# zifeo/distributed-sgd

Hardware: NVIDIA H100
Metric: sgd_samples_per_sec (higher is better)
Workload: dtype f64

## Files before the change

### distributed_sgd_b200/csrc/dsgd_api.cu

```cuda
#include "../../include/dsgd.h"

#include <cuda_runtime.h>
#include <dlfcn.h>
#include <nccl.h>

#include <algorithm>
#include <cstdarg>
#include <cstdio>
#include <cstring>
#include <string>
#include <vector>

#include "dsgd_kernels.cuh"
#include "dsgd_persistent.cuh"
#include "dsgd_stream.cuh"
#include "dsgd_async.cuh"
#include <cstdlib>

using namespace dsgd;

struct dsgd_ctx {
  int device = 0;
  int32_t dim = 0;
  double lambda = 0.0;
// ... 10 lines not shown
  int64_t n_rows = 0, nnz = 0, n_pairs = 0;
  bool rows_unique = false;
  uint32_t *rp16 = nullptr;
  uint2 *pairs = nullptr;
  int8_t *label = nullptr;
  float *yabs = nullptr;

  double *w = nullptr, *g = nullptr, *d = nullptr, *w_req = nullptr;
  float *w32 = nullptr, *w32_req = nullptr;
  unsigned long long *n_exact = nullptr;
  bool stream_ready = false;
  double *scal = nullptr;
  unsigned long long *cnt = nullptr;
  double *partial = nullptr;
  double *out2 = nullptr;
  double *gsum = nullptr;
  std::vector<int32_t> worker_counts;
  int32_t n_local = 1, k_total = 0;
  bool have_d = false;

  int32_t *samples = nullptr;
  int64_t samples_cap = 0, samples_n = 0;
  double *losses = nullptr;
  int64_t losses_cap = 0;
  double *preds = nullptr;
  int64_t preds_cap = 0;

  ncclComm_t comm = nullptr;

  double *p_wbuf[2] = {nullptr, nullptr};
  double *p_gbuf[3] = {nullptr, nullptr, nullptr};
  double2 *p_rec[3] = {nullptr, nullptr, nullptr};
  unsigned long long *p_acc = nullptr;
  unsigned *p_hinge = nullptr;
  int64_t p_hinge_cap = 0;
  unsigned *p_bar = nullptr;
  bool p_ready = false;
  long long *p_tl = nullptr;

  cudaStream_t astream = nullptr;
  cudaStream_t stream2 = nullptr;
  double *m_w = nullptr;
  double *outbox = nullptr;
  double *peer_w[kMaxReplicas] = {};
  bool peer_ipc[kMaxReplicas] = {};
  int *a_stop = nullptr;
  unsigned long long *a_cnt = nullptr;
  double *a_scratch = nullptr;
  int64_t a_scratch_lanes = 0;
  int32_t *a_rows = nullptr, *a_assigned = nullptr, *a_replay = nullptr;
  int64_t a_rows_cap = 0, a_assigned_cap = 0, a_replay_cap = 0;
  int32_t *u_idx = nullptr; double *u_val = nullptr; int64_t u_cap = 0;
  bool a_running = false;
  cudaEvent_t a_ev0 = nullptr, a_ev1 = nullptr;

  double *xblk = nullptr;
  double *peer_x[kMaxWorld] = {};
  bool peer_x_ipc[kMaxWorld] = {};
  int grid_limit = 0;
  int64_t x_step = 0;
  int64_t x_steps_run = 0;
  unsigned long long *x_llw = nullptr;
  unsigned long long *x_stats = nullptr;

  int32_t prof_every = 0;
  int64_t prof_seen = 0;
  std::vector<std::pair<cudaEvent_t, cudaEvent_t>> prof_events;
  size_t prof_used = 0;

  mutable std::string err;
  mutable std::string info;
};

static thread_local std::string g_create_err;

struct nccl_api {
  ncclResult_t (*GetUniqueId)(ncclUniqueId *) = nullptr;
  ncclResult_t (*CommInitRank)(ncclComm_t *, int, ncclUniqueId, int) = nullptr;
  ncclResult_t (*AllReduce)(const void *, void *, size_t, ncclDataType_t, ncclRedOp_t, ncclComm_t, cudaStream_t) = nullptr;
  ncclResult_t (*CommDestroy)(ncclComm_t) = nullptr;
  const char *(*GetErrorString)(ncclResult_t) = nullptr;
  bool ok = false;
  std::string why;
};
static nccl_api &nccl() {
  static nccl_api api = [] {
    nccl_api a;
    void *h = dlopen("libnccl.so.2", RTLD_NOW | RTLD_NOLOAD);
    if (!h)
      if (const char *p = getenv("DSGD_NCCL_PATH")) h = dlopen(p, RTLD_NOW | RTLD_GLOBAL);
    if (!h) h = dlopen("libnccl.so.2", RTLD_NOW | RTLD_GLOBAL);
    if (!h) { a.why = std::string("cannot load libnccl.so.2: ") + dlerror(); return a; }
// ... 111 lines not shown
  if ((e = cudaMalloc(&ctx->out2, sizeof(double) * 8)) != cudaSuccess) return bail("cudaMalloc out2", e);
  if ((e = cudaMalloc(&ctx->gsum, vd)) != cudaSuccess) return bail("cudaMalloc gsum", e);
  cudaMemsetAsync(ctx->gsum, 0, vd, ctx->stream);
  cudaMemsetAsync(ctx->w, 0, vd, ctx->stream);
  cudaMemsetAsync(ctx->g, 0, vd, ctx->stream);
  cudaMemsetAsync(ctx->d, 0, vd, ctx->stream);
  cudaMemsetAsync(ctx->w_req, 0, vd, ctx->stream);
  cudaMemsetAsync(ctx->w32, 0, sizeof(float) * (size_t)(dim + 2), ctx->stream);
  cudaMemsetAsync(ctx->scal, 0, sizeof(double) * kNumScal, ctx->stream);
  cudaMemsetAsync(ctx->cnt, 0, sizeof(unsigned long long) * kNumCnt, ctx->stream);
  if ((e = cudaStreamSynchronize(ctx->stream)) != cudaSuccess) return bail("init memset", e);
  *out = ctx;
  return DSGD_OK;
}

extern "C" int dsgd_destroy(dsgd_ctx *ctx) {
  if (!ctx) return DSGD_OK;
  cudaSetDevice(ctx->device);
  cudaDeviceSynchronize();
  if (ctx->comm) nccl().CommDestroy(ctx->comm);
  for (int r = 0; r < kMaxReplicas; ++r)
    if (ctx->peer_w[r] && ctx->peer_ipc[r]) cudaIpcCloseMemHandle(ctx->peer_w[r]);
  for (int r = 0; r < kMaxWorld; ++r)
    if (ctx->peer_x[r] && ctx->peer_x_ipc[r]) cudaIpcCloseMemHandle(ctx->peer_x[r]);
  if (ctx->xblk) cudaFree(ctx->xblk);
  if (ctx->x_llw) cudaFree(ctx->x_llw);
  void *aptrs[] = {ctx->m_w, ctx->outbox, ctx->a_stop, ctx->a_cnt, ctx->a_scratch, ctx->a_rows, ctx->a_assigned, ctx->a_replay, ctx->u_idx, ctx->u_val};
  for (void *q : aptrs) if (q) cudaFree(q);
  if (ctx->a_ev0) { cudaEventDestroy(ctx->a_ev0); cudaEventDestroy(ctx->a_ev1); }
  if (ctx->astream) cudaStreamDestroy(ctx->astream);
  if (ctx->stream2) cudaStreamDestroy(ctx->stream2);
  void *ptrs[] = {ctx->rp16, ctx->pairs, ctx->label, ctx->yabs, ctx->w, ctx->g, ctx->d, ctx->w_req, ctx->w32, ctx->w32_req, ctx->n_exact, ctx->scal,
                  ctx->cnt, ctx->partial, ctx->out2, ctx->gsum, ctx->p_wbuf[0], ctx->p_wbuf[1], ctx->p_gbuf[0],
                  ctx->p_gbuf[1], ctx->p_gbuf[2], ctx->p_rec[0], ctx->p_rec[1], ctx->p_rec[2], ctx->p_acc, ctx->p_hinge, ctx->p_bar, ctx->x_stats, ctx->samples,
                  ctx->losses, ctx->preds};
  for (void *p : ptrs) if (p) cudaFree(p);
  if (ctx->ev0) cudaEventDestroy(ctx->ev0);
  if (ctx->ev1) cudaEventDestroy(ctx->ev1);
  for (auto &pe : ctx->prof_events) { cudaEventDestroy(pe.first); cudaEventDestroy(pe.second); }
  if (ctx->own_stream) cudaStreamDestroy(ctx->own_stream);
  delete ctx;
  return DSGD_OK;
}

extern "C" const char *dsgd_last_error(const dsgd_ctx *ctx) { return ctx ? ctx->err.c_str() : g_create_err.c_str(); }

extern "C" const char *dsgd_info(const dsgd_ctx *ctx) {
  if (!ctx) return "{}";
  char buf[512];
  snprintf(buf, sizeof buf,
           "{\"device\": %d, \"name\": \"%s\", \"sm_count\": %d, \"arch\": \"sm_90a\", \"dim\": %d, \"rank\": %d, "
           "\"world\": %d, \"n_rows\": %lld, \"nnz\": %lld, \"state_dtype\": \"f64\", \"value_dtype\": \"f32\"}",
           ctx->device, ctx->dev_name.c_str(), ctx->sm_count, ctx->dim, ctx->rank, ctx->world, (long long)ctx->n_rows,
           (long long)ctx->nnz);
  ctx->info = buf;
  return ctx->info.c_str();
}

extern "C" int dsgd_set_stream(dsgd_ctx *ctx, void *cuda_stream) {
  if (!ctx) return DSGD_ERR_INVALID;
  CU(cudaSetDevice(ctx->device));
  CU(cudaStreamSynchronize(ctx->stream));
  ctx->stream = cuda_stream ? (cudaStream_t)cuda_stream : ctx->own_stream;
  return DSGD_OK;
}

extern "C" int dsgd_synchronize(dsgd_ctx *ctx) {
// ... 396 lines not shown
  CU(cudaSetDevice(ctx->device));
  CU(cudaStreamSynchronize(ctx->stream));
  CU(cudaMemcpy(&host, ctx->n_exact, sizeof host, cudaMemcpyDeviceToHost));
  *rows = (int64_t)host;
  return DSGD_OK;
}


extern "C" int dsgd_comm_unique_id(uint8_t id[DSGD_UNIQUE_ID_BYTES]) {
  static_assert(sizeof(ncclUniqueId) == DSGD_UNIQUE_ID_BYTES, "ncclUniqueId size");
  if (!id) return DSGD_ERR_INVALID;
  if (!nccl().ok) return fail(nullptr, DSGD_ERR_NCCL, "%s", nccl().why.c_str());
  ncclUniqueId u;
  ncclResult_t r = nccl().GetUniqueId(&u);
  if (r != ncclSuccess) return fail(nullptr, DSGD_ERR_NCCL, "ncclGetUniqueId: %s", nccl().GetErrorString(r));
  memcpy(id, &u, sizeof u);
  return DSGD_OK;
}

extern "C" int dsgd_comm_init(dsgd_ctx *ctx, const uint8_t id[DSGD_UNIQUE_ID_BYTES]) {
  if (!ctx) return DSGD_ERR_INVALID;
  NEED(id, DSGD_ERR_INVALID, "dsgd_comm_init: id is NULL");
  NEED(!ctx->comm, DSGD_ERR_STATE, "dsgd_comm_init: communicator already initialised");
  CU(cudaSetDevice(ctx->device));
  ncclUniqueId u;
  memcpy(&u, id, sizeof u);
  NEED(nccl().ok, DSGD_ERR_NCCL, "%s", nccl().why.c_str());
  NC(nccl().CommInitRank(&ctx->comm, ctx->world, u, ctx->rank));
  return DSGD_OK;
}

constexpr int kPCons = 8, kPUpd = 6, kPStages = 8, kPStagePairs = 2560, kPMaxChunks = 128;
using PSmem = PersistSmem<kPCons, kPUpd, kPStages, kPStagePairs, kPMaxChunks>;
#define DSGD_PERSIST_KERNEL(multi) k_sync_persistent<kPCons, kPUpd, kPStages, kPStagePairs, kPMaxChunks, multi>
static bool persist_timeline() { static const bool v = getenv("DSGD_PERSIST_TIMELINE") != nullptr; return v; }

static int persist_prepare(dsgd_ctx *ctx, int64_t n_steps) {
  if (!ctx->p_ready) {
    const size_t vd = sizeof(double) * (size_t)(ctx->dim + 2);
    for (int i = 0; i < 2; ++i) CU(cudaMalloc(&ctx->p_wbuf[i], vd));
    for (int i = 0; i < 3; ++i) {
      CU(cudaMalloc(&ctx->p_gbuf[i], vd));
      CU(cudaMemsetAsync(ctx->p_gbuf[i], 0, vd, ctx->stream));
      CU(cudaMalloc(&ctx->p_rec[i], 2 * vd));
      CU(cudaMemsetAsync(ctx->p_rec[i], 0, 2 * vd, ctx->stream));
    }
    CU(cudaMalloc(&ctx->p_acc, sizeof(unsigned long long) * 3 * kAccStride));
    CU(cudaMalloc(&ctx->p_bar, sizeof(unsigned) * 4));
    CU(cudaFuncSetAttribute((const void *)DSGD_PERSIST_KERNEL(false), cudaFuncAttributeMaxDynamicSharedMemorySize, (int)sizeof(PSmem)));
    CU(cudaFuncSetAttribute((const void *)DSGD_PERSIST_KERNEL(true), cudaFuncAttributeMaxDynamicSharedMemorySize, (int)sizeof(PSmem)));
    ctx->p_ready = true;
  }
  if (ctx->p_hinge_cap < n_steps) {
    if (ctx->p_hinge) CU(cudaFree(ctx->p_hinge));
    ctx->p_hinge = nullptr;
    const int64_t want = std::max<int64_t>(n_steps, 4096);
    CU(cudaMalloc(&ctx->p_hinge, sizeof(unsigned) * (size_t)want));
    ctx->p_hinge_cap = want;
  }
  return DSGD_OK;
}

static int persist_grid(const dsgd_ctx *ctx, int64_t batch) {
  const int g = ctx->grid_limit > 0 ? std::min(ctx->grid_limit, ctx->sm_count) : ctx->sm_count;
  if (cdiv(batch, kMaxRowsPerCta) > g) return 0;
  if (ctx->n_pairs >= (1ll << 31)) return 0;
  return g;
}
static bool persist_multi_fits(const dsgd_ctx *ctx, int G) {
  const int slice = (cdiv(ctx->dim + 1, G) + 31) & ~31;
  return slice <= (kPCons + kPUpd) * 32;
}

static cudaError_t persist_launch(dsgd_ctx *ctx, void *fn, int G, void **args) {
  if (ctx->grid_limit > 0) return cudaLaunchKernel(fn, dim3(G), dim3((kPCons + kPUpd + 1) * 32), args, sizeof(PSmem), ctx->stream);
  return cudaLaunchCooperativeKernel(fn, dim3(G), dim3((kPCons + kPUpd + 1) * 32), args, sizeof(PSmem), ctx->stream);
}

static int persist_params(dsgd_ctx *ctx, PersistParams &pp, const int32_t *samples_dev, int64_t n_per_step, int64_t n_steps,
                          double lr, double *losses_dev, int G) {
  (void)G;
  memset(&pp, 0, sizeof pp);
  pp.rp16 = ctx->rp16; pp.pairs = ctx->pairs; pp.label = ctx->label; pp.samples = samples_dev;
  pp.n_steps = n_steps; pp.batch = (int32_t)n_per_step; pp.dim = ctx->dim;
  pp.wbuf[0] = ctx->p_wbuf[0]; pp.wbuf[1] = ctx->p_wbuf[1];
  for (int i = 0; i < 3; ++i) { pp.gbuf[i] = ctx->p_gbuf[i]; pp.rec[i] = ctx->p_rec[i]; }
  pp.d = ctx->d; pp.acc = ctx->p_acc; pp.bar = ctx->p_bar; pp.hinge = ctx->p_hinge; pp.losses = losses_dev;
  pp.w_out = ctx->w; pp.w32_out = ctx->w32; pp.scal = ctx->scal;
  pp.abort_flag = reinterpret_cast<int *>(ctx->p_bar + 1);
  CU(cudaMemsetAsync(ctx->p_acc, 0, sizeof(unsigned long long) * 3 * kAccStride, ctx->stream));
  pp.lambda = ctx->lambda; pp.lr = lr; pp.world = 1;
  CU(cudaMemsetAsync(ctx->p_hinge, 0, sizeof(unsigned) * (size_t)n_steps, ctx->stream));
  CU(cudaMemsetAsync(ctx->p_bar, 0, sizeof(unsigned) * 4, ctx->stream));
  if (persist_timeline()) {
    if (!ctx->p_tl) CU(cudaMalloc(&ctx->p_tl, sizeof(long long) * kTlWords));
    CU(cudaMemsetAsync(ctx->p_tl, 0, sizeof(long long) * kTlWords, ctx->stream));
    pp.tl = ctx->p_tl;
  }
  return DSGD_OK;
}

static int persist_run(dsgd_ctx *ctx, const int32_t *samples_dev, int64_t n_per_step, int64_t n_steps, double lr,
                       double *losses_dev) {
  int rc = persist_prepare(ctx, n_steps);
  if (rc) return rc;
  const int G = persist_grid(ctx, n_per_step);
  NEED((uint64_t)G * (uint64_t)(n_steps + 2) < (1ull << 32), DSGD_ERR_INVALID, "dsgd_sync_steps: too many steps for one launch");
  PersistParams pp;
  if ((rc = persist_params(ctx, pp, samples_dev, n_per_step, n_steps, lr, losses_dev, G))) return rc;
  k_rec_init<<<cdiv(ctx->dim, 256), 256, 0, ctx->stream>>>(ctx->w, ctx->dim, ctx->p_rec[0], ctx->p_rec[1], ctx->p_rec[2]);
  LAUNCHED();
  pp.k_den = 1.0;
  pp.timeout_cycles = 4000000000ll;
  void *args[] = {&pp};
  auto *pe = prof_slot(ctx);
  if (pe) cudaEventRecord(pe->first, ctx->stream);
  CU(persist_launch(ctx, (void *)DSGD_PERSIST_KERNEL(false), G, args));
  if (pe) cudaEventRecord(pe->second, ctx->stream);
  LAUNCHED();
  return DSGD_OK;
}

static size_t xblk_stride(const dsgd_ctx *ctx) { return (size_t)(ctx->dim + kReplicaPad); }
static size_t xblk_words(const dsgd_ctx *ctx) { return ((size_t)ctx->dim + 1 + 31) / 32; }
static size_t xblk_bm_offset(const dsgd_ctx *ctx) { return 2 * (size_t)kMaxWorld * 2 * xblk_stride(ctx); }
static size_t xblk_doubles(const dsgd_ctx *ctx) { return xblk_bm_offset(ctx) + (size_t)kMaxWorld * 2 * xblk_words(ctx); }

static int xblk_ensure(dsgd_ctx *ctx) {
  if (ctx->xblk) return DSGD_OK;
  CU(cudaSetDevice(ctx->device));
  CU(cudaMalloc(&ctx->xblk, sizeof(double) * xblk_doubles(ctx)));
  CU(cudaMemset(ctx->xblk, 0, sizeof(double) * xblk_doubles(ctx)));
  CU(cudaMalloc(&ctx->x_stats, sizeof(unsigned long long) * 4));
  CU(cudaMemset(ctx->x_stats, 0, sizeof(unsigned long long) * 4));
  return DSGD_OK;
}

static int xllw_ensure(dsgd_ctx *ctx) {
  if (ctx->x_llw) return DSGD_OK;
  CU(cudaMalloc(&ctx->x_llw, 2 * 2 * sizeof(unsigned long long) * xblk_stride(ctx)));
  CU(cudaMemsetAsync(ctx->x_llw, 0, 2 * 2 * sizeof(unsigned long long) * xblk_stride(ctx), ctx->stream));
  return DSGD_OK;
}

static bool xchg_complete(const dsgd_ctx *ctx) {
  if (ctx->world <= 1 || ctx->world > kMaxWorld || !ctx->xblk) return false;
  for (int r = 0; r < ctx->world; ++r)
    if (r != ctx->rank && !ctx->peer_x[r]) return false;
  return true;
}

static int persist_run_multi(dsgd_ctx *ctx, const int32_t *samples_dev, int64_t n_per_step, int64_t n_steps, double lr,
                             double *losses_dev) {
  int rc = persist_prepare(ctx, n_steps);
  if (rc) return rc;
  const int G = persist_grid(ctx, n_per_step);
  NEED((uint64_t)G * (uint64_t)(n_steps + 2) < (1ull << 32), DSGD_ERR_INVALID, "dsgd_sync_steps: too many steps for one launch");
  PersistParams pp;
  if ((rc = persist_params(ctx, pp, samples_dev, n_per_step, n_steps, lr, losses_dev, G))) return rc;
  CU(cudaMemcpyAsync(ctx->p_wbuf[0], ctx->w, sizeof(double) * (size_t)ctx->dim, cudaMemcpyDeviceToDevice, ctx->stream));
  pp.k_den = (double)ctx->world;
  pp.timeout_cycles = 20000000000ll;
  pp.world = ctx->world; pp.rank = ctx->rank; pp.step_base = ctx->x_step;
  pp.xstride = (int)xblk_stride(ctx);
  pp.xwords = (int)xblk_words(ctx);
  for (int r = 0; r < ctx->world; ++r) {
    unsigned long long *blk = reinterpret_cast<unsigned long long *>((r == ctx->rank) ? ctx->xblk : ctx->peer_x[r]);
    pp.xval[r] = blk;
    pp.xbm[r] = blk + xblk_bm_offset(ctx);
  }
  if ((rc = xllw_ensure(ctx))) return rc;
  pp.llw[0] = ctx->x_llw;
  pp.llw[1] = ctx->x_llw + 2 * xblk_stride(ctx);
  pp.xstats = ctx->x_stats;
  void *args[] = {&pp};
  auto *pe = prof_slot(ctx);
  if (pe) cudaEventRecord(pe->first, ctx->stream);
  CU(persist_launch(ctx, (void *)DSGD_PERSIST_KERNEL(true), G, args));
  if (pe) cudaEventRecord(pe->second, ctx->stream);
  LAUNCHED();
  ctx->x_step += n_steps + 6;
  ctx->x_steps_run += n_steps;
  return DSGD_OK;
}

extern "C" int dsgd_reserve(dsgd_ctx *ctx, int64_t n_samples, int64_t n_steps) {
  if (!ctx) return DSGD_ERR_INVALID;
  NEED(n_samples >= 0 && n_steps >= 0, DSGD_ERR_INVALID, "dsgd_reserve: negative size");
  CU(cudaSetDevice(ctx->device));
  int rc = ensure_i32(ctx, &ctx->samples, &ctx->samples_cap, n_samples);
  if (rc) return rc;
  if ((rc = ensure_f64(ctx, &ctx->losses, &ctx->losses_cap, n_steps))) return rc;
  if ((rc = persist_prepare(ctx, n_steps))) return rc;
  if (persist_timeline() && !ctx->p_tl) CU(cudaMalloc(&ctx->p_tl, sizeof(long long) * kTlWords));
  if (ctx->world > 1 && !(ctx->flags & DSGD_FLAG_ASYNC)) {
    if ((rc = xblk_ensure(ctx))) return rc;
    if ((rc = xllw_ensure(ctx))) return rc;
  }
  CU(cudaStreamSynchronize(ctx->stream));
  return DSGD_OK;
}

extern "C" int dsgd_set_grid_limit(dsgd_ctx *ctx, int32_t n_ctas) {
  if (!ctx) return DSGD_ERR_INVALID;
  NEED(n_ctas >= 0, DSGD_ERR_INVALID, "dsgd_set_grid_limit: negative");
  ctx->grid_limit = n_ctas;
  return DSGD_OK;
}

extern "C" int dsgd_xchg_stats(dsgd_ctx *ctx, int64_t *value_words, int64_t *bitmap_words, int64_t *steps) {
  if (!ctx) return DSGD_ERR_INVALID;
  unsigned long long host[2] = {0, 0};
  if (ctx->x_stats) {
    CU(cudaSetDevice(ctx->device));
    CU(cudaStreamSynchronize(ctx->stream));
    CU(cudaMemcpy(host, ctx->x_stats, sizeof host, cudaMemcpyDeviceToHost));
  }
  if (value_words) *value_words = (int64_t)host[0];
  if (bitmap_words) *bitmap_words = (int64_t)host[1];
  if (steps) *steps = ctx->x_steps_run;
  return DSGD_OK;
}

extern "C" int dsgd_xchg_export(dsgd_ctx *ctx, uint8_t handle[DSGD_IPC_HANDLE_BYTES]) {
  if (!ctx || !handle) return DSGD_ERR_INVALID;
  NEED(!(ctx->flags & DSGD_FLAG_ASYNC), DSGD_ERR_STATE, "dsgd_xchg_export: ctx is in async mode");
// ... 10 lines not shown
  NEED(peer_rank >= 0 && peer_rank < ctx->world && peer_rank < kMaxWorld && peer_rank != ctx->rank, DSGD_ERR_INVALID,
       "dsgd_xchg_import: bad peer rank %d", peer_rank);
  int rc = xblk_ensure(ctx);
  if (rc) return rc;
  cudaIpcMemHandle_t h;
  memcpy(&h, handle, sizeof h);
  void *ptr = nullptr;
  CU(cudaIpcOpenMemHandle(&ptr, h, cudaIpcMemLazyEnablePeerAccess));
  if (ctx->peer_x[peer_rank] && ctx->peer_x_ipc[peer_rank]) cudaIpcCloseMemHandle(ctx->peer_x[peer_rank]);
  ctx->peer_x[peer_rank] = static_cast<double *>(ptr);
  ctx->peer_x_ipc[peer_rank] = true;
  return DSGD_OK;
}

extern "C" int dsgd_xchg_attach(dsgd_ctx *ctx, int peer_rank, dsgd_ctx *peer) {
  if (!ctx || !peer) return DSGD_ERR_INVALID;
  NEED(peer_rank >= 0 && peer_rank < ctx->world && peer_rank < kMaxWorld && peer_rank != ctx->rank, DSGD_ERR_INVALID,
       "dsgd_xchg_attach: bad peer rank %d", peer_rank);
  NEED(peer->dim == ctx->dim, DSGD_ERR_INVALID, "dsgd_xchg_attach: dimension mismatch");
  int rc = xblk_ensure(ctx);
  if (rc) return rc;
  if ((rc = xblk_ensure(peer))) { ctx->err = peer->err; return rc; }
  CU(cudaSetDevice(ctx->device));
  if (peer->device != ctx->device) {
    int can = 0;
    CU(cudaDeviceCanAccessPeer(&can, ctx->device, peer->device));
    NEED(can, DSGD_ERR_CUDA, "dsgd_xchg_attach: device %d cannot access device %d", ctx->device, peer->device);
    cudaError_t e = cudaDeviceEnablePeerAccess(peer->device, 0);
    if (e != cudaSuccess && e != cudaErrorPeerAccessAlreadyEnabled) CU(e);
    (void)cudaGetLastError();
  }
  ctx->peer_x[peer_rank] = peer->xblk;
  ctx->peer_x_ipc[peer_rank] = false;
  return DSGD_OK;
}

static int persist_check(dsgd_ctx *ctx) {
  if (!ctx->p_ready) return DSGD_OK;
  unsigned host[2] = {0, 0};
  CU(cudaMemcpy(host, ctx->p_bar, sizeof host, cudaMemcpyDeviceToHost));
  NEED(host[1] == 0, DSGD_ERR_TIMEOUT, "persistent sync kernel: a device-side wait (grid barrier, peer word) hit its watchdog");
  return DSGD_OK;
}

static_assert(kTlWords == DSGD_TIMELINE_WORDS, "timeline layout");
extern "C" int dsgd_debug_timeline(dsgd_ctx *ctx, long long *out) {
  if (!ctx || !out) return DSGD_ERR_INVALID;
  NEED(ctx->p_tl, DSGD_ERR_STATE, "no timeline recorded (set DSGD_PERSIST_TIMELINE=1)");
  CU(cudaStreamSynchronize(ctx->stream));
  CU(cudaMemcpy(out, ctx->p_tl, sizeof(long long) * kTlWords, cudaMemcpyDeviceToHost));
  return DSGD_OK;
}

extern "C" int dsgd_set_workers(dsgd_ctx *ctx, int32_t n_local, const int32_t *counts, int32_t k_total) {
  if (!ctx) return DSGD_ERR_INVALID;
  NEED(n_local >= 0 && k_total >= 0, DSGD_ERR_INVALID, "dsgd_set_workers: negative count");
  NEED(n_local <= 1 || counts, DSGD_ERR_INVALID, "dsgd_set_workers: counts is NULL");
  std::vector<int32_t> c;
  if (counts)
    for (int32_t v = 0; v < n_local; ++v) {
      NEED(counts[v] > 0, DSGD_ERR_EMPTY, "dsgd_set_workers: worker %d has an empty batch (Vec.sum of an empty list throws)", v);
      c.push_back(counts[v]);
    }
  ctx->worker_counts = c;
  ctx->n_local = n_local;
  ctx->k_total = k_total;
// ... 394 lines not shown
```

### distributed_sgd_b200/csrc/dsgd_persistent.cuh

```cuda
#pragma once
#include <cuda_runtime.h>
#include <stdint.h>

#include "dsgd_kernels.cuh"

namespace dsgd {

constexpr int kMaxWorld = 8;

struct PersistParams {
  const uint32_t *rp16;
  const uint2 *pairs;
  const int8_t *label;
  const int32_t *samples;
  int64_t n_steps;
  int32_t batch;
  int32_t dim;
  double *wbuf[2];
  double *gbuf[3];
  double2 *rec[3];
  const double *d;
  unsigned long long *acc;
  unsigned *hinge;
  double *losses;
  double *w_out;
  float *w32_out;
  double *scal;
  unsigned *bar;
  int *abort_flag;
  double lambda, lr, k_den;
  long long timeout_cycles;
  long long *tl;
  int world, rank;
  int64_t step_base;
  unsigned long long *xval[kMaxWorld];
  unsigned long long *xbm[kMaxWorld];
  int xstride, xwords;
  unsigned long long *llw[2];
  unsigned long long *xstats;
};
static_assert(sizeof(PersistParams) <= 4000, "kernel parameter space is 4 KB");

__device__ __forceinline__ uint32_t smem_u32(const void *p) { return (uint32_t)__cvta_generic_to_shared(p); }
__device__ __forceinline__ void mbar_init(uint64_t *b, unsigned count) {
  asm volatile("mbarrier.init.shared::cta.b64 [%0], %1;" ::"r"(smem_u32(b)), "r"(count) : "memory");
}
__device__ __forceinline__ void mbar_expect_tx(uint64_t *b, unsigned bytes) {
  asm volatile("mbarrier.arrive.expect_tx.shared::cta.b64 _, [%0], %1;" ::"r"(smem_u32(b)), "r"(bytes) : "memory");
}
__device__ __forceinline__ void mbar_arrive(uint64_t *b) {
  asm volatile("mbarrier.arrive.shared::cta.b64 _, [%0];" ::"r"(smem_u32(b)) : "memory");
}
__device__ __forceinline__ void bulk_g2s(void *dst, const void *src, unsigned bytes, uint64_t *b) {
  asm volatile("cp.async.bulk.shared::cluster.global.mbarrier::complete_tx::bytes [%0], [%1], %2, [%3];" ::"r"(
                   smem_u32(dst)),
               "l"(src), "r"(bytes), "r"(smem_u32(b))
// ... 95 lines not shown
    }
  }
  return ok;
}

constexpr int kAccStride = 16;
__device__ __forceinline__ void red_add_u64(unsigned long long *p, unsigned long long v) {
  asm volatile("red.relaxed.gpu.global.add.u64 [%0], %1;" ::"l"(p), "l"(v) : "memory");
}
__device__ __forceinline__ void acc_push_one(unsigned long long *slot3, unsigned long long *ovf, double v) {
  if (!(fabs(v) < 4503599627370496.0)) {
    red_add_u64(ovf, 1ull);
    return;
  }
  const double a = fabs(v);
  const double f2 = floor(a);
  const double r1 = (a - f2) * 1099511627776.0;
  const double f1 = floor(r1);
  const double r0 = rint((r1 - f1) * 1099511627776.0);
  const bool neg = v < 0.0;
  auto put = [&](unsigned long long *dst, double limb) {
    if (limb != 0.0) {
      const unsigned long long u = (unsigned long long)(long long)limb;
      red_add_u64(dst, neg ? (0ull - u) : u);
    }
  };
  put(slot3 + 0, r0);
  put(slot3 + 1, f1);
  put(slot3 + 2, f2);
}
__device__ __forceinline__ void acc_push(unsigned long long *acc, double sd, double sn) {
  acc_push_one(acc + 0, acc + 6, sd);
  acc_push_one(acc + 3, acc + 6, sn);
}
__device__ __forceinline__ void acc_read(const unsigned long long *acc, int lane, double &sd, double &sn) {
  unsigned long long q0 = 0, q1 = 0;
  if (lane < 4)
    asm volatile("ld.relaxed.gpu.global.v2.u64 {%0, %1}, [%2];" : "=l"(q0), "=l"(q1) : "l"(acc + 2 * lane) : "memory");
  long long l[7];
#pragma unroll
  for (int i = 0; i < 7; ++i) l[i] = (long long)__shfl_sync(0xffffffffu, (i & 1) ? q1 : q0, i >> 1);
  const double nan = __longlong_as_double(0x7ff8000000000000ll);
  sd = ((double)l[0] * 0x1p-80 + (double)l[1] * 0x1p-40) + (double)l[2];
  sn = ((double)l[3] * 0x1p-80 + (double)l[4] * 0x1p-40) + (double)l[5];
  if (l[6] != 0) { sd = nan; sn = nan; }
}

constexpr int kChunkPairs = 128;
constexpr uint32_t kChunkGlobal = 1u << 31;
constexpr int kMaxRowsPerCta = 32;

template <int kMaxChunks>
struct StageMeta {
  int n_rows;
  int n_chunks;
  int n_multi;
  int n_pairs;
  int row_y[kMaxRowsPerCta];
  uint32_t row_b[kMaxRowsPerCta];
  int row_len[kMaxRowsPerCta];
  short row_first[kMaxRowsPerCta];
  short row_nch[kMaxRowsPerCta];
  uint32_t ch_off[kMaxChunks];
  short ch_n[kMaxChunks];
  short ch_row[kMaxChunks];
  double part[kMaxChunks];
// ... 173 lines not shown
          const double gvv = filt(filt((double)__uint_as_float(pr.y)) * y);
          if (gvv != 0.0) red_add_f64(gbase + (size_t)gstride * pr.x, gvv);
        }
      }
    }
  }
  for (int m = warp; m < mt.n_rows; m += kCons) {
    const int nch = mt.row_nch[m];
    if (nch == 0) {
      if (lane == 0) hinge += 1u;
    } else if (nch < 0) {
      const uint2 *grow = pairs + (size_t)mt.row_b[m] * 2;
      const int len = mt.row_len[m];
      double acc = 0.0;
      for (int k = lane; k < len; k += 32) {
        const uint2 pr = __ldg(&grow[k]);
        acc += filt(filt((double)__uint_as_float(pr.y)) * fetch.get1(pr.x));
      }
      const double dot = warp_sum(acc);
      const int yi = mt.row_y[m];
      const double y = (double)yi;
      if (lane == 0) hinge += (unsigned)(1 - yi * pred_of(dot));
      if (!(y * dot < 0.0))
        for (int k = lane; k < len; k += 32) {
          const uint2 pr = __ldg(&grow[k]);
          const double gvv = filt(filt((double)__uint_as_float(pr.y)) * y);
          if (gvv != 0.0) red_add_f64(gbase + (size_t)gstride * pr.x, gvv);
        }
    }
  }
  return hinge;
}

template <int kCons, int kUpd, int kStages, int kStagePairs, int kMaxChunks, bool kMulti>
__global__ void __launch_bounds__((kCons + kUpd + 1) * 32, 1) k_sync_persistent(const PersistParams p) {
  using Smem = PersistSmem<kCons, kUpd, kStages, kStagePairs, kMaxChunks>;
  extern __shared__ __align__(128) unsigned char smem_raw[];
  Smem &sm = *reinterpret_cast<Smem *>(smem_raw);

  const int lane = threadIdx.x & 31;
  const int warp = threadIdx.x >> 5;
  const bool is_cons = warp < kCons;
  const bool is_upd = warp >= kCons && warp < kCons + kUpd;
  const int G = gridDim.x;
  const int B = p.batch;
  const int64_t S = p.n_steps;
  constexpr int kSyncThreads = (kCons + kUpd) * 32;
  const int n_r = (B > (int)blockIdx.x) ? (B - 1 - (int)blockIdx.x) / G + 1 : 0;

  if (threadIdx.x == 0) {
    for (int s = 0; s < kStages; ++s) {
      mbar_init(&sm.full[s], 1u);
      mbar_init(&sm.empty[s], (unsigned)kCons);
    }
    mbar_init(&sm.c_bar[0], 1u);
    mbar_init(&sm.c_bar[1], 1u);
    mbar_init(&sm.u_bar, (unsigned)(kMulti ? kCons + kUpd : kUpd));
    sm.c_val[0] = 0.0;
    sm.nrm_val[0] = 0.0;
    sm.hinge_acc = 0u;
    sm.ok = 1;
  }
  asm volatile("fence.mbarrier_init.release.cluster;" ::: "memory");
  __syncthreads();
  if (threadIdx.x == 0) mbar_arrive(&sm.c_bar[0]);

  if (!is_cons && !is_upd) {
// ... 52 lines not shown
      const int listed_chunks = __reduce_max_sync(0xffffffffu, (lane < n_r && listed) ? (my_chunk + nch) : 0);
      const unsigned multi = __ballot_sync(0xffffffffu, lane < n_r && listed && nch > 1);
      if (lane == 31) mt.n_pairs = ps;
      if (lane == 0) {
        mt.n_rows = n_r;
        mt.n_chunks = listed_chunks;
        mt.n_multi = __popc(multi);
      }
      __syncwarp();
      if (lane == 0) {
        if (ring_bytes) mbar_expect_tx(&sm.full[st], ring_bytes);
        else mbar_arrive(&sm.full[st]);
      }
      __syncwarp();
      if (my_bytes) bulk_g2s(&sm.ring[st][my_pair], p.pairs + (size_t)b0 * 2, my_bytes, &sm.full[st]);
      b0 = b1; e0 = e1; y0 = y1;
      load_win(id_next, b1, e1, y1);
      id_next = load_id(t + 3);
    }
    return;
  }

  const double lr = p.lr;
  const int64_t base = kMulti ? p.step_base : 0;
  unsigned phase = 0;
  const int n_upd = G * kUpd * 32;
  const int u0 = blockIdx.x * kUpd * 32 + ((int)threadIdx.x - kCons * 32);
  const int K = p.world, me = p.rank;
  const int slice = ((p.dim + 1 + G - 1) / G + 31) & ~31;
  const int j_col = blockIdx.x * slice + (int)threadIdx.x;
  const bool col_act = kMulti && (int)threadIdx.x < slice && j_col <= p.dim;
  const int col_word = j_col >> 5;
  unsigned long long st_val = 0, st_bm = 0;
  constexpr int kUpdCols = 2;
  double wreg[kUpdCols], dreg[kUpdCols];
  int ttl[kUpdCols];
  bool gnz[kUpdCols];
#pragma unroll
  for (int i = 0; i < kUpdCols; ++i) {
    wreg[i] = dreg[i] = 0.0;
    ttl[i] = 0;
    gnz[i] = false;
    if constexpr (!kMulti) {
      const int j = u0 + i * n_upd;
      if (is_upd && j < p.dim) { wreg[i] = __ldcg(&p.rec[2][j].x); dreg[i] = __ldg(&p.d[j]); }
    }
  }
  if constexpr (kMulti) {
    if (col_act && j_col < p.dim) { wreg[0] = __ldcg(&p.wbuf[0][j_col]); dreg[0] = __ldg(&p.d[j_col]); }
  }

  int gi_prev = (int)((base + 2) % 3), gi_cur = (int)(base % 3), gi_next = (int)((base + 1) % 3);
  int ti_prev = 2, ti_cur = 0, ti_next = 1;
  for (int64_t T = base; T <= base + S; ++T) {
    const int64_t t = T - base;
    const bool first = (t == 0), last = (t == S);
    const double *Gprev = p.gbuf[gi_prev];
    double *Gcur = p.gbuf[gi_cur];
    double *Gzero = p.gbuf[gi_next];
    const unsigned long long *acc_prev = p.acc + (size_t)ti_prev * kAccStride;
    unsigned long long *acc_cur = p.acc + (size_t)ti_cur * kAccStride;
    unsigned long long *acc_next = p.acc + (size_t)ti_next * kAccStride;
    const double2 *Rprev = p.rec[ti_prev];
    double2 *Rcur = p.rec[ti_cur];
    double2 *Rnext = p.rec[ti_next];
    const unsigned c_par = (unsigned)((t >> 1) & 1);
    const bool tl_cta = p.tl && t >= kTlFirst && t < kTlFirst + kTlSteps && blockIdx.x < kTlCtas;
    long long *tl_rec = tl_cta ? p.tl + 256 * 16 + ((t - kTlFirst) * kTlCtas + blockIdx.x) * kTlPerCta : nullptr;
    long long *tl_row = (p.tl && blockIdx.x == 0 && t < 256) ? p.tl + t * 16 : nullptr;
    bool ok = true;
    if (warp == 0) DSGD_TL(0);

    if (warp == kCons && !first) {
      double c_prev, nrm_prev;
      if (kMulti && t == 1) {
        c_prev = p.scal[kScalC];
        nrm_prev = p.scal[kScalNrm2];
      } else {
        double sd, sn;
        acc_read(acc_prev, lane, sd, sn);
        c_prev = p.lambda * 2.0 * sd;
        nrm_prev = sn;
      }
      if (blockIdx.x == 0 && lane < 8) acc_next[lane] = 0ull;
      if (lane == 0) {
        sm.c_val[t & 1] = c_prev;
        sm.nrm_val[t & 1] = nrm_prev;
        mbar_arrive(&sm.c_bar[t & 1]);
        if (!kMulti && p.losses && blockIdx.x == 0)
          p.losses[t - 1] = p.lambda * nrm_prev + (double)__ldcg(&p.hinge[t - 1]) / (double)B;
      }
      __syncwarp();
      DSGD_TL(9);
    }
    double pd = 0.0, pn = 0.0;
    auto publish_partial = [&]() {
      pd = warp_sum(pd);
      pn = warp_sum(pn);
      if (lane == 0) {
        sm.red[warp][0] = pd;
        sm.red[warp][1] = pn;
        mbar_arrive(&sm.u_bar);
      }
      if (warp == kCons) {
        mbar_wait(&sm.u_bar, (unsigned)(t & 1), p.abort_flag, p.timeout_cycles);
        if (lane == 0) {
          double sd = 0.0, sn = 0.0;
#pragma unroll
          for (int i = kMulti ? 0 : kCons; i < kCons + kUpd; ++i) { sd += sm.red[i][0]; sn += sm.red[i][1]; }
          if (sd != 0.0 || sn != 0.0) acc_push(acc_cur, sd, sn);
        }
        __syncwarp();
      }
    };

    if constexpr (kMulti) {
      unsigned long long *LWcur = p.llw[T & 1];
      const int parp = (int)((T + 1) & 1);
      const unsigned gtag = (unsigned)T;
      const unsigned wtag = (unsigned)(T + 1);
      if ((int)threadIdx.x < slice) {
        if (first) {
          if (col_act) {
            if (j_col < p.dim) ll_store(LWcur + 2 * (size_t)j_col, wreg[0], wtag);
            Gzero[j_col] = 0.0;
          }
        } else {
          double own = 0.0;
          if (col_act) {
            own = __ldcg(&Gprev[j_col]);
            if (j_col < p.dim) own = filt(own);
          }
          const unsigned my_bits = __ballot_sync(0xffffffffu, own != 0.0);
          const bool warp_act = blockIdx.x * slice + (warp << 5) <= p.dim;
          if (warp_act) {
            const size_t vslot = 2 * (((size_t)me * 2 + parp) * p.xstride + (size_t)j_col);
            const size_t bslot = ((size_t)me * 2 + parp) * p.xwords + (size_t)col_word;
            for (int k = 0; k < K; ++k) {
              if (k == me) continue;
              if (lane == 0) ll_store32(p.xbm[k] + bslot, my_bits, gtag);
              if (own != 0.0) ll_store(p.xval[k] + vslot, own, gtag);
            }
            if (lane == 0) { st_bm += 1; st_val += (unsigned)__popc(my_bits); }
// ... 119 lines not shown
        if (lane == 0) mbar_arrive(&sm.empty[st]);
        if (warp == 0) DSGD_TL(3);
      }
    } else {
      if (is_cons) {
        if (!last) {
          const int st = (int)t & (kStages - 1);
          auto &mt = sm.meta[st];
          mbar_wait(&sm.full[st], (unsigned)(((unsigned)t / kStages) & 1u), p.abort_flag, p.timeout_cycles);
          if (warp == 0) DSGD_TL(1);
          FetchLocal fetch{Rprev, &sm.c_bar[t & 1], c_par, &sm.c_val[t & 1], p.abort_flag, p.timeout_cycles, p.k_den, lr};
          const unsigned hinge = consume_stage<kCons, kMaxChunks>(mt, &sm.ring[st][0], p.pairs, &Rcur[0].y, 2, fetch, warp,
                                                                            lane, warp == 0 ? tl_row : nullptr);
          if (lane == 0 && hinge) atomicAdd(&sm.hinge_acc, hinge);
          if (tl_rec && warp == 0 && lane == 0) tl_rec[2] = mt.n_pairs;
          __syncwarp();
          if (lane == 0) mbar_arrive(&sm.empty[st]);
          if (warp == 0) DSGD_TL(3);
        }
      } else {
        double gv[kUpdCols];
#pragma unroll
        for (int i = 0; i < kUpdCols; ++i) {
          const int j = u0 + i * n_upd;
          gv[i] = (j < p.dim) ? __ldcg(&Rprev[j].y) : 0.0;
        }
        mbar_wait(&sm.c_bar[t & 1], c_par, p.abort_flag, p.timeout_cycles);
        const double c_prev = *(volatile double *)&sm.c_val[t & 1];
        const bool add_c = (c_prev != 0.0) && (fabs(c_prev) > kEps);
#pragma unroll
        for (int i = 0; i < kUpdCols; ++i) {
          const int j = u0 + i * n_upd;
          if (j < p.dim) {
            if (gv[i] != 0.0) {
              wreg[i] = apply_update(wreg[i], gv[i], c_prev, add_c, p.k_den, lr);
              ttl[i] = 3;
            }
            if (ttl[i] > 0) { Rcur[j].x = wreg[i]; --ttl[i]; }
            if (gnz[i]) Rnext[j].y = 0.0;
            gnz[i] = gv[i] != 0.0;
            pd += filt(wreg[i] * dreg[i]);
            pn += wreg[i] * wreg[i];
          }
        }
        for (int j = u0 + kUpdCols * n_upd; j < p.dim; j += n_upd) {
          const double2 r = __ldcg(&Rprev[j]);
          const double wn = apply_update(r.x, r.y, c_prev, add_c, p.k_den, lr);
          Rcur[j].x = wn;
          Rnext[j].y = 0.0;
          pd += filt(wn * __ldg(&p.d[j]));
          pn += wn * wn;
        }
        if (warp == kCons) DSGD_TL(10);
        publish_partial();
      }
    }

    if (!ok) *(volatile int *)&sm.ok = 0;
    if (tl_row && lane == 0) sm.tl_warp[warp] = clock64();
    named_bar_sync(3, kSyncThreads);
    ++phase;
    if (threadIdx.x == 0) {
      if (tl_row) {
        long long mc = 0, mu = 0;
        for (int i = 0; i < kCons; ++i) mc = max(mc, sm.tl_warp[i]);
        for (int i = kCons; i < kCons + kUpd; ++i) mu = max(mu, sm.tl_warp[i]);
        tl_row[13] = mc;
        tl_row[14] = mu;
      }
      if (!last) {
        const unsigned h = sm.hinge_acc;
        if constexpr (kMulti) {
          if (h) red_add_f64(&Gcur[p.dim], (double)h);
          if (blockIdx.x == 0) red_add_f64(&Gcur[p.dim], (double)B * 4294967296.0);
        } else {
          if (h) atomicAdd(&p.hinge[t], h);
        }
        sm.hinge_acc = 0u;
      }
      if (tl_rec) tl_rec[0] = global_ns();
      else if (tl_row) tl_row[6] = clock64();
      bool bar_ok = grid_barrier_arrive_wait(p.bar, phase * (unsigned)G, p.abort_flag, p.timeout_cycles);
      if (*(volatile int *)&sm.ok == 0) { *(volatile int *)p.abort_flag = 1; bar_ok = false; }
      sm.ok = bar_ok ? 1 : 0;
      if (tl_rec) tl_rec[1] = global_ns();
      else if (tl_row) tl_row[7] = clock64();
    }
    named_bar_sync(3, kSyncThreads);
    if (*(volatile int *)&sm.ok == 0) return;
    { const int a = gi_prev; gi_prev = gi_cur; gi_cur = gi_next; gi_next = a; }
    { const int a = ti_prev; ti_prev = ti_cur; ti_cur = ti_next; ti_next = a; }
  }

  if (blockIdx.x == 0 && warp == kCons && S > 0) {
    double sd, sn;
    acc_read(p.acc + (size_t)ti_prev * kAccStride, lane, sd, sn);
    if (lane == 0) { p.scal[kScalC] = p.lambda * 2.0 * sd; p.scal[kScalNrm2] = sn; }
  }
  if constexpr (kMulti) {
    const unsigned long long *LW = p.llw[(base + S) & 1];
    const unsigned wtag = (unsigned)(base + S + 1);
    const int n_all = G * kSyncThreads;
    for (int j = blockIdx.x * kSyncThreads + threadIdx.x; j < p.dim; j += n_all) {
      double wv = 0.0;
      ll_try_load(LW + 2 * (size_t)j, wtag, wv);
      p.w_out[j] = wv;
      p.w32_out[j] = (float)wv;
    }
    if (p.xstats && lane == 0 && (st_val | st_bm)) {
      atomicAdd(&p.xstats[0], st_val);
      atomicAdd(&p.xstats[1], st_bm);
    }
  } else if (is_upd) {
    const double2 *Rfin = p.rec[ti_prev];
#pragma unroll
    for (int i = 0; i < kUpdCols; ++i) {
      const int j = u0 + i * n_upd;
      if (j < p.dim) { p.w_out[j] = wreg[i]; p.w32_out[j] = (float)wreg[i]; }
    }
    for (int j = u0 + kUpdCols * n_upd; j < p.dim; j += n_upd) {
      const double wv = __ldcg(&Rfin[j]).x;
      p.w_out[j] = wv;
      p.w32_out[j] = (float)wv;
    }
  }
}

__global__ void __launch_bounds__(256) k_rec_init(const double *__restrict__ w, int dim, double2 *__restrict__ rec0,
                                                  double2 *__restrict__ rec1, double2 *__restrict__ rec2) {
  const int j = blockIdx.x * blockDim.x + threadIdx.x;
// ... 10 lines not shown
```

Measured before the change: 70.62 million.

## Defer loss norm accumulation off critical path and template update column count

Moves the per-step norm and hinge loss accumulation out of the grid-barrier critical path. The norm push is deferred one step into a separate loss-term accumulator and the hinge is added after the barrier. Losses are read two steps late into a triple-buffered area, which replaces the per-step hinge array and its memset. Also templates the kernel on register-held update columns (2/4/8, chosen from dim and grid), packs per-column ttl/gnz flags into one bitfield, and uses cooperative launch unless the GPU is shared. This adds complexity in the loss bookkeeping and NaN propagation.

Result: no change. 71.00 million (median of 6 runs) (+0.5%).

```diff
diff --git a/distributed_sgd_b200/csrc/dsgd_api.cu b/distributed_sgd_b200/csrc/dsgd_api.cu
--- a/distributed_sgd_b200/csrc/dsgd_api.cu
+++ b/distributed_sgd_b200/csrc/dsgd_api.cu
@@ -66,8 +66,6 @@
   double *p_gbuf[3] = {nullptr, nullptr, nullptr};
   double2 *p_rec[3] = {nullptr, nullptr, nullptr};
   unsigned long long *p_acc = nullptr;
-  unsigned *p_hinge = nullptr;
-  int64_t p_hinge_cap = 0;
   unsigned *p_bar = nullptr;
   bool p_ready = false;
   long long *p_tl = nullptr;
@@ -92,6 +90,7 @@
   double *peer_x[kMaxWorld] = {};
   bool peer_x_ipc[kMaxWorld] = {};
   int grid_limit = 0;
+  bool shares_gpu = false;
   int64_t x_step = 0;
   int64_t x_steps_run = 0;
   unsigned long long *x_llw = nullptr;
@@ -269,7 +268,7 @@
   if (ctx->stream2) cudaStreamDestroy(ctx->stream2);
   void *ptrs[] = {ctx->rp16, ctx->pairs, ctx->label, ctx->yabs, ctx->w, ctx->g, ctx->d, ctx->w_req, ctx->w32, ctx->w32_req, ctx->n_exact, ctx->scal,
                   ctx->cnt, ctx->partial, ctx->out2, ctx->gsum, ctx->p_wbuf[0], ctx->p_wbuf[1], ctx->p_gbuf[0],
-                  ctx->p_gbuf[1], ctx->p_gbuf[2], ctx->p_rec[0], ctx->p_rec[1], ctx->p_rec[2], ctx->p_acc, ctx->p_hinge, ctx->p_bar, ctx->x_stats, ctx->samples,
+                  ctx->p_gbuf[1], ctx->p_gbuf[2], ctx->p_rec[0], ctx->p_rec[1], ctx->p_rec[2], ctx->p_acc, ctx->p_bar, ctx->x_stats, ctx->samples,
                   ctx->losses, ctx->preds};
   for (void *p : ptrs) if (p) cudaFree(p);
   if (ctx->ev0) cudaEventDestroy(ctx->ev0);
@@ -732,10 +731,16 @@
 
 constexpr int kPCons = 8, kPUpd = 6, kPStages = 8, kPStagePairs = 2560, kPMaxChunks = 128;
 using PSmem = PersistSmem<kPCons, kPUpd, kPStages, kPStagePairs, kPMaxChunks>;
-#define DSGD_PERSIST_KERNEL(multi) k_sync_persistent<kPCons, kPUpd, kPStages, kPStagePairs, kPMaxChunks, multi>
+#define DSGD_PERSIST_KERNEL(multi, cols) k_sync_persistent<kPCons, kPUpd, kPStages, kPStagePairs, kPMaxChunks, multi, cols>
+static const void *persist_kernel_single(int dim, int G) {
+  const int cols = cdiv(dim, (int64_t)kPUpd * 32 * G);
+  if (cols <= 2) return (const void *)DSGD_PERSIST_KERNEL(false, 2);
+  if (cols <= 4) return (const void *)DSGD_PERSIST_KERNEL(false, 4);
+  return (const void *)DSGD_PERSIST_KERNEL(false, 8);
+}
 static bool persist_timeline() { static const bool v = getenv("DSGD_PERSIST_TIMELINE") != nullptr; return v; }
 
-static int persist_prepare(dsgd_ctx *ctx, int64_t n_steps) {
+static int persist_prepare(dsgd_ctx *ctx) {
   if (!ctx->p_ready) {
     const size_t vd = sizeof(double) * (size_t)(ctx->dim + 2);
     for (int i = 0; i < 2; ++i) CU(cudaMalloc(&ctx->p_wbuf[i], vd));
@@ -745,18 +750,12 @@
       CU(cudaMalloc(&ctx->p_rec[i], 2 * vd));
       CU(cudaMemsetAsync(ctx->p_rec[i], 0, 2 * vd, ctx->stream));
     }
-    CU(cudaMalloc(&ctx->p_acc, sizeof(unsigned long long) * 3 * kAccStride));
+    CU(cudaMalloc(&ctx->p_acc, sizeof(unsigned long long) * 6 * kAccStride));
     CU(cudaMalloc(&ctx->p_bar, sizeof(unsigned) * 4));
-    CU(cudaFuncSetAttribute((const void *)DSGD_PERSIST_KERNEL(false), cudaFuncAttributeMaxDynamicSharedMemorySize, (int)sizeof(PSmem)));
-    CU(cudaFuncSetAttribute((const void *)DSGD_PERSIST_KERNEL(true), cudaFuncAttributeMaxDynamicSharedMemorySize, (int)sizeof(PSmem)));
+    for (const void *fn : {(const void *)DSGD_PERSIST_KERNEL(false, 2), (const void *)DSGD_PERSIST_KERNEL(false, 4),
+                           (const void *)DSGD_PERSIST_KERNEL(false, 8), (const void *)DSGD_PERSIST_KERNEL(true, 2)})
+      CU(cudaFuncSetAttribute(fn, cudaFuncAttributeMaxDynamicSharedMemorySize, (int)sizeof(PSmem)));
     ctx->p_ready = true;
-  }
-  if (ctx->p_hinge_cap < n_steps) {
-    if (ctx->p_hinge) CU(cudaFree(ctx->p_hinge));
-    ctx->p_hinge = nullptr;
-    const int64_t want = std::max<int64_t>(n_steps, 4096);
-    CU(cudaMalloc(&ctx->p_hinge, sizeof(unsigned) * (size_t)want));
-    ctx->p_hinge_cap = want;
   }
   return DSGD_OK;
 }
@@ -773,7 +772,7 @@
 }
 
 static cudaError_t persist_launch(dsgd_ctx *ctx, void *fn, int G, void **args) {
-  if (ctx->grid_limit > 0) return cudaLaunchKernel(fn, dim3(G), dim3((kPCons + kPUpd + 1) * 32), args, sizeof(PSmem), ctx->stream);
+  if (ctx->grid_limit > 0 && ctx->shares_gpu) return cudaLaunchKernel(fn, dim3(G), dim3((kPCons + kPUpd + 1) * 32), args, sizeof(PSmem), ctx->stream);
   return cudaLaunchCooperativeKernel(fn, dim3(G), dim3((kPCons + kPUpd + 1) * 32), args, sizeof(PSmem), ctx->stream);
 }
 
@@ -785,12 +784,11 @@
   pp.n_steps = n_steps; pp.batch = (int32_t)n_per_step; pp.dim = ctx->dim;
   pp.wbuf[0] = ctx->p_wbuf[0]; pp.wbuf[1] = ctx->p_wbuf[1];
   for (int i = 0; i < 3; ++i) { pp.gbuf[i] = ctx->p_gbuf[i]; pp.rec[i] = ctx->p_rec[i]; }
-  pp.d = ctx->d; pp.acc = ctx->p_acc; pp.bar = ctx->p_bar; pp.hinge = ctx->p_hinge; pp.losses = losses_dev;
+  pp.d = ctx->d; pp.acc = ctx->p_acc; pp.bar = ctx->p_bar; pp.losses = losses_dev;
   pp.w_out = ctx->w; pp.w32_out = ctx->w32; pp.scal = ctx->scal;
   pp.abort_flag = reinterpret_cast<int *>(ctx->p_bar + 1);
-  CU(cudaMemsetAsync(ctx->p_acc, 0, sizeof(unsigned long long) * 3 * kAccStride, ctx->stream));
+  CU(cudaMemsetAsync(ctx->p_acc, 0, sizeof(unsigned long long) * 6 * kAccStride, ctx->stream));
   pp.lambda = ctx->lambda; pp.lr = lr; pp.world = 1;
-  CU(cudaMemsetAsync(ctx->p_hinge, 0, sizeof(unsigned) * (size_t)n_steps, ctx->stream));
   CU(cudaMemsetAsync(ctx->p_bar, 0, sizeof(unsigned) * 4, ctx->stream));
   if (persist_timeline()) {
     if (!ctx->p_tl) CU(cudaMalloc(&ctx->p_tl, sizeof(long long) * kTlWords));
@@ -802,7 +800,7 @@
 
 static int persist_run(dsgd_ctx *ctx, const int32_t *samples_dev, int64_t n_per_step, int64_t n_steps, double lr,
                        double *losses_dev) {
-  int rc = persist_prepare(ctx, n_steps);
+  int rc = persist_prepare(ctx);
   if (rc) return rc;
   const int G = persist_grid(ctx, n_per_step);
   NEED((uint64_t)G * (uint64_t)(n_steps + 2) < (1ull << 32), DSGD_ERR_INVALID, "dsgd_sync_steps: too many steps for one launch");
@@ -815,7 +813,7 @@
   void *args[] = {&pp};
   auto *pe = prof_slot(ctx);
   if (pe) cudaEventRecord(pe->first, ctx->stream);
-  CU(persist_launch(ctx, (void *)DSGD_PERSIST_KERNEL(false), G, args));
+  CU(persist_launch(ctx, const_cast<void *>(persist_kernel_single(ctx->dim, G)), G, args));
   if (pe) cudaEventRecord(pe->second, ctx->stream);
   LAUNCHED();
   return DSGD_OK;
@@ -852,7 +850,7 @@
 
 static int persist_run_multi(dsgd_ctx *ctx, const int32_t *samples_dev, int64_t n_per_step, int64_t n_steps, double lr,
                              double *losses_dev) {
-  int rc = persist_prepare(ctx, n_steps);
+  int rc = persist_prepare(ctx);
   if (rc) return rc;
   const int G = persist_grid(ctx, n_per_step);
   NEED((uint64_t)G * (uint64_t)(n_steps + 2) < (1ull << 32), DSGD_ERR_INVALID, "dsgd_sync_steps: too many steps for one launch");
@@ -876,7 +874,7 @@
   void *args[] = {&pp};
   auto *pe = prof_slot(ctx);
   if (pe) cudaEventRecord(pe->first, ctx->stream);
-  CU(persist_launch(ctx, (void *)DSGD_PERSIST_KERNEL(true), G, args));
+  CU(persist_launch(ctx, (void *)DSGD_PERSIST_KERNEL(true, 2), G, args));
   if (pe) cudaEventRecord(pe->second, ctx->stream);
   LAUNCHED();
   ctx->x_step += n_steps + 6;
@@ -891,7 +889,7 @@
   int rc = ensure_i32(ctx, &ctx->samples, &ctx->samples_cap, n_samples);
   if (rc) return rc;
   if ((rc = ensure_f64(ctx, &ctx->losses, &ctx->losses_cap, n_steps))) return rc;
-  if ((rc = persist_prepare(ctx, n_steps))) return rc;
+  if ((rc = persist_prepare(ctx))) return rc;
   if (persist_timeline() && !ctx->p_tl) CU(cudaMalloc(&ctx->p_tl, sizeof(long long) * kTlWords));
   if (ctx->world > 1 && !(ctx->flags & DSGD_FLAG_ASYNC)) {
     if ((rc = xblk_ensure(ctx))) return rc;
@@ -968,6 +966,7 @@
   }
   ctx->peer_x[peer_rank] = peer->xblk;
   ctx->peer_x_ipc[peer_rank] = false;
+  if (peer->device == ctx->device) ctx->shares_gpu = true;
   return DSGD_OK;
 }
 
diff --git a/distributed_sgd_b200/csrc/dsgd_persistent.cuh b/distributed_sgd_b200/csrc/dsgd_persistent.cuh
--- a/distributed_sgd_b200/csrc/dsgd_persistent.cuh
+++ b/distributed_sgd_b200/csrc/dsgd_persistent.cuh
@@ -21,7 +21,6 @@
   double2 *rec[3];
   const double *d;
   unsigned long long *acc;
-  unsigned *hinge;
   double *losses;
   double *w_out;
   float *w32_out;
@@ -183,6 +182,17 @@
 __device__ __forceinline__ void acc_push(unsigned long long *acc, double sd, double sn) {
   acc_push_one(acc + 0, acc + 6, sd);
   acc_push_one(acc + 3, acc + 6, sn);
+}
+__device__ __forceinline__ void loss_terms_read(const unsigned long long *lt, int lane, double &sn, double &hinge) {
+  unsigned long long q0 = 0, q1 = 0;
+  if (lane < 3)
+    asm volatile("ld.relaxed.gpu.global.v2.u64 {%0, %1}, [%2];" : "=l"(q0), "=l"(q1) : "l"(lt + 2 * lane) : "memory");
+  long long l[5];
+#pragma unroll
+  for (int i = 0; i < 5; ++i) l[i] = (long long)__shfl_sync(0xffffffffu, (i & 1) ? q1 : q0, i >> 1);
+  sn = ((double)l[0] * 0x1p-80 + (double)l[1] * 0x1p-40) + (double)l[2];
+  if (l[3] != 0) sn = __longlong_as_double(0x7ff8000000000000ll);
+  hinge = (double)(unsigned long long)l[4];
 }
 __device__ __forceinline__ void acc_read(const unsigned long long *acc, int lane, double &sd, double &sn) {
   unsigned long long q0 = 0, q1 = 0;
@@ -422,7 +432,7 @@
   return hinge;
 }
 
-template <int kCons, int kUpd, int kStages, int kStagePairs, int kMaxChunks, bool kMulti>
+template <int kCons, int kUpd, int kStages, int kStagePairs, int kMaxChunks, bool kMulti, int kUpdCols>
 __global__ void __launch_bounds__((kCons + kUpd + 1) * 32, 1) k_sync_persistent(const PersistParams p) {
   using Smem = PersistSmem<kCons, kUpd, kStages, kStagePairs, kMaxChunks>;
   extern __shared__ __align__(128) unsigned char smem_raw[];
@@ -541,15 +551,12 @@
   const bool col_act = kMulti && (int)threadIdx.x < slice && j_col <= p.dim;
   const int col_word = j_col >> 5;
   unsigned long long st_val = 0, st_bm = 0;
-  constexpr int kUpdCols = 2;
   double wreg[kUpdCols], dreg[kUpdCols];
-  int ttl[kUpdCols];
-  bool gnz[kUpdCols];
+  static_assert(3 * kUpdCols <= 32, "column state bits");
+  unsigned cst = 0u;
 #pragma unroll
   for (int i = 0; i < kUpdCols; ++i) {
     wreg[i] = dreg[i] = 0.0;
-    ttl[i] = 0;
-    gnz[i] = false;
     if constexpr (!kMulti) {
       const int j = u0 + i * n_upd;
       if (is_upd && j < p.dim) { wreg[i] = __ldcg(&p.rec[2][j].x); dreg[i] = __ldg(&p.d[j]); }
@@ -561,6 +568,8 @@
 
   int gi_prev = (int)((base + 2) % 3), gi_cur = (int)(base % 3), gi_next = (int)((base + 1) % 3);
   int ti_prev = 2, ti_cur = 0, ti_next = 1;
+  double sn_defer = 0.0;
+  bool sd_ovf1 = false, sd_ovf2 = false;
   for (int64_t T = base; T <= base + S; ++T) {
     const int64_t t = T - base;
     const bool first = (t == 0), last = (t == S);
@@ -570,6 +579,9 @@
     const unsigned long long *acc_prev = p.acc + (size_t)ti_prev * kAccStride;
     unsigned long long *acc_cur = p.acc + (size_t)ti_cur * kAccStride;
     unsigned long long *acc_next = p.acc + (size_t)ti_next * kAccStride;
+    unsigned long long *lt_prev = p.acc + (size_t)(3 + ti_prev) * kAccStride;
+    unsigned long long *lt_cur = p.acc + (size_t)(3 + ti_cur) * kAccStride;
+    unsigned long long *lt_next = p.acc + (size_t)(3 + ti_next) * kAccStride;
     const double2 *Rprev = p.rec[ti_prev];
     double2 *Rcur = p.rec[ti_cur];
     double2 *Rnext = p.rec[ti_next];
@@ -590,14 +602,26 @@
         acc_read(acc_prev, lane, sd, sn);
         c_prev = p.lambda * 2.0 * sd;
         nrm_prev = sn;
+        sd_ovf2 = sd_ovf1;
+        sd_ovf1 = sd != sd;
       }
       if (blockIdx.x == 0 && lane < 8) acc_next[lane] = 0ull;
       if (lane == 0) {
         sm.c_val[t & 1] = c_prev;
         sm.nrm_val[t & 1] = nrm_prev;
         mbar_arrive(&sm.c_bar[t & 1]);
-        if (!kMulti && p.losses && blockIdx.x == 0)
-          p.losses[t - 1] = p.lambda * nrm_prev + (double)__ldcg(&p.hinge[t - 1]) / (double)B;
+        if (!kMulti && p.losses && sn_defer != 0.0) acc_push_one(lt_prev, lt_prev + 3, sn_defer);
+      }
+      if constexpr (!kMulti) {
+        if (blockIdx.x == 0) {
+          if (p.losses && t >= 2) {
+            double sn2, h2;
+            loss_terms_read(lt_next, lane, sn2, h2);
+            if (lane == 0) p.losses[t - 2] = sd_ovf2 ? __longlong_as_double(0x7ff8000000000000ll) : p.lambda * sn2 + h2 / (double)B;
+          }
+          __syncwarp();
+          if (lane < 8) lt_next[lane] = 0ull;
+        }
       }
       __syncwarp();
       DSGD_TL(9);
@@ -617,7 +641,12 @@
           double sd = 0.0, sn = 0.0;
 #pragma unroll
           for (int i = kMulti ? 0 : kCons; i < kCons + kUpd; ++i) { sd += sm.red[i][0]; sn += sm.red[i][1]; }
-          if (sd != 0.0 || sn != 0.0) acc_push(acc_cur, sd, sn);
+          if (kMulti || last) {
+            if (sd != 0.0 || sn != 0.0) acc_push(acc_cur, sd, sn);
+          } else {
+            if (sd != 0.0) acc_push_one(acc_cur + 0, acc_cur + 6, sd);
+            sn_defer = sn;
+          }
         }
         __syncwarp();
       }
@@ -803,13 +832,15 @@
         for (int i = 0; i < kUpdCols; ++i) {
           const int j = u0 + i * n_upd;
           if (j < p.dim) {
+            unsigned ttl = (cst >> (3 * i)) & 3u;
+            const bool gnz = (cst >> (3 * i + 2)) & 1u;
             if (gv[i] != 0.0) {
               wreg[i] = apply_update(wreg[i], gv[i], c_prev, add_c, p.k_den, lr);
-              ttl[i] = 3;
+              ttl = 3u;
             }
-            if (ttl[i] > 0) { Rcur[j].x = wreg[i]; --ttl[i]; }
-            if (gnz[i]) Rnext[j].y = 0.0;
-            gnz[i] = gv[i] != 0.0;
+            if (ttl > 0u) { Rcur[j].x = wreg[i]; --ttl; }
+            if (gnz) Rnext[j].y = 0.0;
+            cst = (cst & ~(7u << (3 * i))) | ((ttl | ((gv[i] != 0.0) ? 4u : 0u)) << (3 * i));
             pd += filt(wreg[i] * dreg[i]);
             pn += wreg[i] * wreg[i];
           }
@@ -839,19 +870,18 @@
         tl_row[13] = mc;
         tl_row[14] = mu;
       }
+      const unsigned h = last ? 0u : sm.hinge_acc;
       if (!last) {
-        const unsigned h = sm.hinge_acc;
         if constexpr (kMulti) {
           if (h) red_add_f64(&Gcur[p.dim], (double)h);
           if (blockIdx.x == 0) red_add_f64(&Gcur[p.dim], (double)B * 4294967296.0);
-        } else {
-          if (h) atomicAdd(&p.hinge[t], h);
         }
         sm.hinge_acc = 0u;
       }
       if (tl_rec) tl_rec[0] = global_ns();
       else if (tl_row) tl_row[6] = clock64();
       bool bar_ok = grid_barrier_arrive_wait(p.bar, phase * (unsigned)G, p.abort_flag, p.timeout_cycles);
+      if (!kMulti && h && p.losses) red_add_u64(lt_cur + 4, h);
       if (*(volatile int *)&sm.ok == 0) { *(volatile int *)p.abort_flag = 1; bar_ok = false; }
       sm.ok = bar_ok ? 1 : 0;
       if (tl_rec) tl_rec[1] = global_ns();
@@ -867,6 +897,11 @@
     double sd, sn;
     acc_read(p.acc + (size_t)ti_prev * kAccStride, lane, sd, sn);
     if (lane == 0) { p.scal[kScalC] = p.lambda * 2.0 * sd; p.scal[kScalNrm2] = sn; }
+    if (!kMulti && p.losses) {
+      double sn1, h1;
+      loss_terms_read(p.acc + (size_t)(3 + ti_next) * kAccStride, lane, sn1, h1);
+      if (lane == 0) p.losses[S - 1] = sd_ovf1 ? __longlong_as_double(0x7ff8000000000000ll) : p.lambda * sn1 + h1 / (double)B;
+    }
   }
   if constexpr (kMulti) {
     const unsigned long long *LW = p.llw[(base + S) & 1];
```
